# qkniep/alpenglow

Measured on AMD Instinct MI355X. Metric: GiB/s device-resident RS shred encode+reconstruct, batched 1 MiB blocks, higher is better.
Workload: dtype u8 (GF(2^16) symbols, bitsliced u32 planes); 1 GPU; 4096 x 1 MiB blocks per GPU, 32:32 encode + reconstruct with 16/32 data shreds erased; blocks_per_gpu=4096, block_bytes=1048576, data_shreds=32, coding_shreds=32, erased_data_shreds=16, lost_coding_shreds=0, random_patterns=False, parallelism=blocks sharded over 1 GPU(s), no collective, only=both

## Files before the change

### alpenglow_amd/csrc/rs_api.cpp

```cpp
#include <hip/hip_runtime.h>

#include <algorithm>
#include <chrono>
#include <cstddef>
#include <cstdlib>
#include <cstring>
#include <new>
#include <utility>
#include <vector>

#include "../../include/alpenglow_rs.h"
#include "gf16.hpp"
#include "rs_ctx.hpp"
#include "rs_launch.hpp"
#include "rs_patterns.hpp"

using namespace ag::host;
using ag::lowrate_chunk;
using ag::mc_chunk;
using ag::padded_shard;
using ag::xform_points;

namespace {

// ... 218 lines not shown
  return AG_RS_OK;
}

int ag_rs_ctx_set_stream(ag_rs_ctx* c, void* s) {
  if (!c) return AG_RS_ERR_INVALID_ARGUMENT;
  return switch_stream(c, static_cast<hipStream_t>(s));
}

int ag_rs_ctx_reset_stream(ag_rs_ctx* c) {
  if (!c) return AG_RS_ERR_INVALID_ARGUMENT;
  return switch_stream(c, c->own_stream);
}

void* ag_rs_ctx_stream(ag_rs_ctx* c) { return c ? static_cast<void*>(c->stream) : nullptr; }

int ag_rs_ctx_synchronize(ag_rs_ctx* c) {
  if (!c) return AG_RS_ERR_INVALID_ARGUMENT;
  if (c->enter()) return AG_RS_ERR_DEVICE;
  return hipStreamSynchronize(c->stream) == hipSuccess ? AG_RS_OK : AG_RS_ERR_DEVICE;
}

int ag_rs_use_high_rate(size_t k, size_t m) {
  const int hr = ag::use_high_rate(k, m);
  return hr < 0 ? -AG_RS_ERR_UNSUPPORTED_SHARD_COUNT : hr;
}

int ag_rs_internal_last_decode_classes(ag_rs_ctx* c, uint64_t* out16) {
  if (!c || !out16) return AG_RS_ERR_INVALID_ARGUMENT;
  std::memcpy(out16, c->last_classes, sizeof c->last_classes);
  return AG_RS_OK;
}

int ag_rs_internal_last_window_kernels(ag_rs_ctx* c, uint32_t* out) {
  if (!c || !out) return AG_RS_ERR_INVALID_ARGUMENT;
  *out = c->last_window_kernels;
  return AG_RS_OK;
}

int ag_rs_internal_server_jobs(ag_rs_ctx* c, uint64_t* out4) {
  if (!c || !out4) return AG_RS_ERR_INVALID_ARGUMENT;
  std::copy(std::begin(c->server_jobs), std::end(c->server_jobs), out4);
  return AG_RS_OK;
}

int ag_rs_internal_fail_next_server_job(ag_rs_ctx* c) {
  if (!c) return AG_RS_ERR_INVALID_ARGUMENT;
  c->fail_next_server_job = true;
  return AG_RS_OK;
}

int ag_rs_internal_last_encode_kernels(ag_rs_ctx* c, uint32_t* out) {
  if (!c || !out) return AG_RS_ERR_INVALID_ARGUMENT;
  *out = c->last_encode_kernels;
  return AG_RS_OK;
}

int ag_rs_internal_last_merkle_kernels(ag_rs_ctx* c, uint32_t* out) {
  if (!c || !out) return AG_RS_ERR_INVALID_ARGUMENT;
  *out = c->last_merkle_kernels;
  return AG_RS_OK;
}

int ag_rs_internal_last_exact_rerun(ag_rs_ctx* c, uint64_t out[2]) {
  if (!c || !out) return AG_RS_ERR_INVALID_ARGUMENT;
  out[0] = c->last_rerun_slices;
  out[1] = c->last_rerun_passes;
  return AG_RS_OK;
}

int ag_rs_has_fast_path(size_t k, size_t m, size_t S) {
  if (S == 0 || S % 2) return 0;
  const size_t Sp = padded_shard(S);
  return xform_points(k, m, Sp) || mc_chunk(k, m, Sp) || lowrate_chunk(k, m, Sp) ? 1 : 0;
}

int ag_rs_encode_batch(ag_rs_ctx* c, size_t k, size_t m, size_t S, size_t nblocks, const uint8_t* orig,
                       size_t ostride, uint8_t* rec, size_t rstride, int memory) {
  if (!c || (nblocks && (!orig || !rec))) return AG_RS_ERR_INVALID_ARGUMENT;
  int st = check_geometry(k, m, S);
  if (st) return st;
  if (ostride < k * S || rstride < m * S) return AG_RS_ERR_INVALID_ARGUMENT;
  if ((st = c->enter())) return st;
  c->last_encode_kernels = 0;
  if (memory == AG_RS_MEM_DEVICE) return encode_device(c, k, m, S, nblocks, orig, ostride, rec, rstride);
  if (memory != AG_RS_MEM_HOST) return AG_RS_ERR_INVALID_ARGUMENT;
  const size_t in_b = k * S, out_b = m * S;
  const size_t group = std::max<size_t>(1, kStageGroupBytes / (in_b + out_b));
  if ((st = c->ensure_copy_streams())) return st;
  size_t g = 0;
  for (size_t b0 = 0; b0 < nblocks; b0 += group, ++g) {
    const size_t n = std::min(group, nblocks - b0);
    auto& sl = c->slot[g & 1];
    AG_HIP(hipStreamWaitEvent(c->h2d, sl.down, 0));
    if ((st = sl.in.ensure(group * in_b, c->h2d)) || (st = sl.out.ensure(group * out_b, c->h2d))) return st;
    AG_HIP(hipMemcpy2DAsync(sl.in.ptr, in_b, orig + b0 * ostride, ostride, in_b, n, hipMemcpyHostToDevice, c->h2d));
    AG_HIP(hipEventRecord(sl.up, c->h2d));
    AG_HIP(hipStreamWaitEvent(c->stream, sl.up, 0));
    if ((st = encode_device(c, k, m, S, n, sl.in.as<uint8_t>(), in_b, sl.out.as<uint8_t>(), out_b))) break;
    AG_HIP(hipEventRecord(sl.done, c->stream));
    AG_HIP(hipStreamWaitEvent(c->d2h, sl.done, 0));
    AG_HIP(hipMemcpy2DAsync(rec + b0 * rstride, rstride, sl.out.ptr, out_b, out_b, n, hipMemcpyDeviceToHost, c->d2h));
    AG_HIP(hipEventRecord(sl.down, c->d2h));
  }
  AG_HIP(hipStreamSynchronize(c->stream));
  AG_HIP(hipStreamSynchronize(c->d2h));
  return st;
// ... 302 lines not shown
```

### alpenglow_amd/csrc/rs_ctx.hpp

```cpp
#pragma once
#include <hip/hip_runtime.h>

#include <chrono>
#include <cstddef>
#include <cstdint>
#include <memory>
#include <type_traits>
#include <utility>
#include <vector>

#include "../../include/alpenglow_rs.h"
#include "cipher.hpp"
#include "gf16.hpp"
#include "rs_launch.hpp"

#define AG_HIP(expr)                                  \
  do {                                                \
    if ((expr) != hipSuccess) return AG_RS_ERR_DEVICE; \
  } while (0)

namespace ag {
namespace host __attribute__((visibility("hidden"))) {

struct DevBuf {
// ... 113 lines not shown
  template <typename T>
  int host(size_t bytes, T** out) {
    if (ev) AG_HIP(hipEventSynchronize(ev));
    else AG_HIP(hipEventCreateWithFlags(&ev, hipEventDisableTiming));
    const int st = pin.ensure(bytes);
    *out = pin.as<T>();
    return st;
  }
  int send(size_t bytes, hipStream_t stream, void* dst = nullptr) {
    if (!dst) {
      const int st = dev.ensure(bytes, stream);
      if (st) return st;
      dst = dev.ptr;
    }
    AG_HIP(hipMemcpyAsync(dst, pin.ptr, bytes, hipMemcpyHostToDevice, stream));
    AG_HIP(hipEventRecord(ev, stream));
    return AG_RS_OK;
  }
};

}
}

using ag::host::DevBuf;
using ag::host::PinBuf;
using ag::host::StagedUpload;
using ag::host::UploadCache;

struct ag_rs_ctx {
  int device = 0;
  hipStream_t own_stream = nullptr;
  hipStream_t stream = nullptr;
  bool tables_ready = false;
  DevBuf d_exp, d_log, d_skew, d_log_walsh;
  DevBuf scratch;
  DevBuf d_flags, d_loc, d_blocks;
  UploadCache<uint64_t> mask;
  UploadCache<uint64_t> stage_mask;
  UploadCache<uint64_t> xmask;
  size_t xmask_w = 0;
  bool xmask_poly = false;
  DevBuf d_rows, d_xblocks;
  UploadCache<uint64_t> x128;
  DevBuf d_rows128;
  std::vector<uint32_t> x128_ids;
  UploadCache<uint8_t> syn;
  DevBuf d_synblocks;
  UploadCache<uint8_t> corr;
  DevBuf d_corrk, d_corrblocks;
  static constexpr int kClassSlots = 16;
  uint64_t last_classes[kClassSlots] = {};
  int decode_depth = 0;
  uint32_t last_encode_kernels = 0;
  uint32_t last_window_kernels = 0;
  DevBuf d_empty_roots;
  DevBuf d_merkle_nodes;
  uint32_t last_merkle_kernels = 0;
  StagedUpload leaf_sizes;
  StagedUpload block_meta;
  DevBuf d_aon_lens, d_aon_digests, d_aon_keys;
  DevBuf d_aon_lens2;
  hipStream_t side = nullptr;
  hipEvent_t side_fork = nullptr, side_join = nullptr;
  DevBuf d_slice_meta;
  DevBuf stage_pad;
  StagedUpload lens;
  DevBuf d_strip;
  DevBuf d_reenc_mask;
  DevBuf d_pipe_few, d_pipe_mask;
  StagedUpload present;
  PinBuf h_strip;
  PinBuf h_slice_meta;
  PinBuf h_pipe_meta;
  StagedUpload rerun;
  uint64_t last_rerun_slices = 0, last_rerun_passes = 0;
  DevBuf d_ed_base;
  static constexpr int kPipeBufs = 37;
  DevBuf pipe[kPipeBufs];
  DevBuf d_sh_roots, d_sh_commit, d_sh_onvalid, d_sh_list;
  DevBuf d_intake;
  StagedUpload intake_win;
  PinBuf h_intake;
  DevBuf d_repair;
  StagedUpload repair_blocks;
  PinBuf h_repair;
  DevBuf d_block;
  StagedUpload block_cols;
  PinBuf h_block;
  struct Slot {
    DevBuf in, out;
    hipEvent_t up = nullptr, done = nullptr, down = nullptr;
  } slot[2];
  hipStream_t h2d = nullptr, d2h = nullptr;
  DevBuf one_in, one_out;
  ag::LatencyMailbox* mb = nullptr;
  ag::LatencyMailbox* mb_dev = nullptr;
  hipStream_t server_stream = nullptr;
  uint32_t server_seq = 0;
  uint32_t server_p_seq = 0, server_dp_seq = 0;
  bool server_broken = false;
  bool fail_next_server_job = false;
  uint64_t server_jobs[4] = {};
  std::vector<PinBuf> abandoned_pins;

  void forget_uploads() {
    mask.key.clear();
    stage_mask.key.clear();
    xmask.key.clear();
    x128.key.clear();
    syn.key.clear();
    corr.key.clear();
  }

  int enter() { return hipSetDevice(device) == hipSuccess ? AG_RS_OK : AG_RS_ERR_DEVICE; }

  int ensure_tables() {
    if (tables_ready) return AG_RS_OK;
    const ag::Gf16Tables& t = ag::gf16_tables();
    std::vector<uint16_t> lw(t.log, t.log + ag::kGfOrder);
    lw[0] = 0;
    for (size_t dist = 1; dist < ag::kGfOrder; dist <<= 1)
      for (size_t r = 0; r < ag::kGfOrder; r += 2 * dist)
        for (size_t i = r; i < r + dist; ++i) {
          const uint32_t a = lw[i], b = lw[i + dist];
          const uint32_t s = a + b, d = a - b;
          lw[i] = static_cast<uint16_t>(s + (s >> 16));
          lw[i + dist] = static_cast<uint16_t>(d + (d >> 16));
        }
    int st;
    if ((st = d_exp.ensure(sizeof t.exp, stream)) || (st = d_log.ensure(sizeof t.log, stream)) ||
        (st = d_skew.ensure(sizeof t.skew, stream)) || (st = d_log_walsh.ensure(lw.size() * 2, stream)))
      return st;
    AG_HIP(hipMemcpy(d_exp.ptr, t.exp, sizeof t.exp, hipMemcpyHostToDevice));
    AG_HIP(hipMemcpy(d_log.ptr, t.log, sizeof t.log, hipMemcpyHostToDevice));
    AG_HIP(hipMemcpy(d_skew.ptr, t.skew, sizeof t.skew, hipMemcpyHostToDevice));
    AG_HIP(hipMemcpy(d_log_walsh.ptr, lw.data(), lw.size() * 2, hipMemcpyHostToDevice));
    tables_ready = true;
    return AG_RS_OK;
  }

  ag::GfDeviceTables dtables() const {
    return {d_exp.as<uint16_t>(), d_log.as<uint16_t>(), d_skew.as<uint16_t>(), d_log_walsh.as<uint16_t>()};
  }

  int ensure_side_stream() {
    if (side) return AG_RS_OK;
    AG_HIP(hipStreamCreateWithFlags(&side, hipStreamNonBlocking));
    AG_HIP(hipEventCreateWithFlags(&side_fork, hipEventDisableTiming));
    AG_HIP(hipEventCreateWithFlags(&side_join, hipEventDisableTiming));
    return AG_RS_OK;
  }

  int ensure_copy_streams() {
    if (h2d) return AG_RS_OK;
    AG_HIP(hipStreamCreateWithFlags(&h2d, hipStreamNonBlocking));
    AG_HIP(hipStreamCreateWithFlags(&d2h, hipStreamNonBlocking));
    for (Slot& s : slot) {
      AG_HIP(hipEventCreateWithFlags(&s.up, hipEventDisableTiming));
      AG_HIP(hipEventCreateWithFlags(&s.done, hipEventDisableTiming));
      AG_HIP(hipEventCreateWithFlags(&s.down, hipEventDisableTiming));
      AG_HIP(hipEventRecord(s.down, d2h));
    }
    return AG_RS_OK;
  }

  void server_stop() {
    if (!mb) return;
    (void)hipSetDevice(device);
// ... 130 lines not shown
```

### alpenglow_amd/csrc/rs_dispatch.cpp

```cpp
#include <hip/hip_runtime.h>

#include <algorithm>
#include <cstring>
#include <vector>

#include "gf16.hpp"
#include "rs_ctx.hpp"
#include "rs_launch.hpp"
#include "rs_patterns.hpp"
#include "shredder.hpp"

namespace ag {
namespace host {

int check_geometry(size_t k, size_t m, size_t S) {
  if (use_high_rate(k, m) < 0) return AG_RS_ERR_UNSUPPORTED_SHARD_COUNT;
  if (S == 0 || S % 2) return AG_RS_ERR_INVALID_SHARD_SIZE;
  if (S > 0xFFFFFFFEull) return AG_RS_ERR_INVALID_ARGUMENT;
  return AG_RS_OK;
}

bool odd_layout(const void* a, const void* b, size_t sa, size_t sb) {
  return ((reinterpret_cast<uintptr_t>(a) | reinterpret_cast<uintptr_t>(b) | sa | sb) & 1) != 0;
}
// ... 13 lines not shown
  p.rec = rec;
  p.rec_block_stride = rstride;
  p.rec_shard_stride = sstride;
  return p;
}

XformParams xform_params(const uint8_t* in, size_t in_stride, size_t n_in, uint8_t* out, size_t out_stride,
                         size_t n_out, size_t sstride, size_t cps, size_t nblocks) {
  XformParams p{};
  p.in = in;
  p.in_block_stride = in_stride;
  p.in_shard_stride = sstride;
  p.out = out;
  p.out_block_stride = out_stride;
  p.out_shard_stride = sstride;
  p.n_in = static_cast<uint32_t>(n_in);
  p.n_out = static_cast<uint32_t>(n_out);
  p.chunks_per_shard = static_cast<uint32_t>(cps);
  p.total_columns = static_cast<uint64_t>(nblocks) * cps;
  return p;
}

int encode_restrided(ag_rs_ctx* c, size_t k, size_t m, size_t Sv, size_t sstride, size_t off, size_t nblocks,
                     const uint8_t* orig, size_t ostride, uint8_t* rec, size_t rstride) {
  const size_t Sp = padded_shard(Sv), per_block = (k + m) * Sp;
  const size_t group = std::max<size_t>(1, kRestrideGroupBytes / per_block);
  int st = c->stage_pad.ensure(std::min(group, nblocks) * per_block, c->stream);
  if (st) return st;
  c->last_encode_kernels |= kEkRestride;
  uint8_t* pad = c->stage_pad.as<uint8_t>();
  for (size_t b0 = 0; b0 < nblocks; b0 += group) {
    const size_t nb = std::min(group, nblocks - b0);
    if (launch_restride(orig + b0 * ostride + off, ostride, sstride, pad, per_block, Sp, static_cast<uint32_t>(Sv),
                        static_cast<uint32_t>(k), nb, false, nullptr, false, c->stream) != hipSuccess)
      return AG_RS_ERR_DEVICE;
    if ((st = encode_device(c, k, m, Sp, nb, pad, per_block, pad + k * Sp, per_block))) return st;
    if (launch_restride(pad + k * Sp, per_block, Sp, rec + b0 * rstride + off, rstride, sstride,
                        static_cast<uint32_t>(Sv), static_cast<uint32_t>(m), nb, true, nullptr, false,
                        c->stream) != hipSuccess)
      return AG_RS_ERR_DEVICE;
  }
  return AG_RS_OK;
}

int encode_cols(ag_rs_ctx* c, size_t k, size_t m, size_t S, size_t sstride, size_t nblocks, const uint8_t* orig,
                size_t ostride, uint8_t* rec, size_t rstride) {
  const unsigned npts = xform_points(k, m, S);
  const unsigned mc = mc_chunk(k, m, S);
  const unsigned lr = lowrate_chunk(k, m, S);
  if (npts || mc || lr) {
    const XformParams p = xform_params(orig, ostride, k, rec, rstride, m, sstride, S / 64, nblocks);
    hipError_t e = hipSuccess;
    if (npts) {
      c->last_encode_kernels |= npts == 32 ? encode32_kernel(p) : kEkXformH8;
      e = launch_xform(npts == 32 ? XformKind::kEncode32 : XformKind::kEncode64, p, c->stream);
    } else if (mc) {
      c->last_encode_kernels |= kEkEncodeMc;
      e = launch_encode_mc(mc, p, c->stream);
    } else {
      for (size_t j = 0; j * lr < m && e == hipSuccess;) {
        XformParams pj = p;
        pj.out = rec + j * lr * sstride;
        if (lr == 32 && j % 2 == 0 && (j + 1) * lr < m && j < 4) {
          pj.n_out = static_cast<uint32_t>(std::min<size_t>(2 * lr, m - j * lr));
          c->last_encode_kernels |= kEkLowRate2;
          e = launch_xform_lowrate2(static_cast<unsigned>(j / 2), pj, c->stream);
          j += 2;
          continue;
        }
        pj.n_out = static_cast<uint32_t>(std::min<size_t>(lr, m - j * lr));
        c->last_encode_kernels |= kEkLowRate;
        e = launch_xform_lowrate(lr, static_cast<unsigned>(j), pj, c->stream);
        ++j;
      }
    }
    return e == hipSuccess ? AG_RS_OK : AG_RS_ERR_DEVICE;
  }
  int st = c->ensure_tables();
  if (st) return st;
  const int hr = use_high_rate(k, m);
  const size_t chunk = hr ? next_pow2(m) : next_pow2(k);
  const size_t cover = hr ? k : m;
  const size_t rows = std::max(chunk, (cover + chunk - 1) / chunk * chunk);
  const size_t nsym = S / 2;
  const size_t per_block = rows * nsym * 2;
  const size_t per_launch = std::max<size_t>(1, kGenericScratchBytes / per_block);
  if ((st = c->scratch.ensure(std::min(per_launch, nblocks) * per_block, c->stream))) return st;
  for (size_t b0 = 0; b0 < nblocks; b0 += per_launch) {
    auto p = shard_params<GenericEncodeParams>(orig + b0 * ostride, ostride, rec + b0 * rstride, rstride, sstride);
    p.k = static_cast<uint32_t>(k);
    p.m = static_cast<uint32_t>(m);
    p.high_rate = static_cast<uint32_t>(hr);
    p.chunk = static_cast<uint32_t>(chunk);
    p.rows = static_cast<uint32_t>(rows);
    p.shard_bytes = static_cast<uint32_t>(S);
    p.nsym = static_cast<uint32_t>(nsym);
    p.nblocks = std::min(per_launch, nblocks - b0);
    p.scratch = c->scratch.as<uint16_t>();
    p.t = c->dtables();
    c->last_encode_kernels |= kEkGeneric;
    if (launch_generic_encode(p, c->stream) != hipSuccess) return AG_RS_ERR_DEVICE;
  }
  return AG_RS_OK;
}

XformParams tail_params(const uint8_t* in, size_t in_stride, size_t n_in, uint8_t* out, size_t out_stride,
                        size_t n_out, size_t S, size_t nblocks) {
  XformParams p = xform_params(in, in_stride, n_in, out, out_stride, n_out, S, padded_shard(S) / 64, nblocks);
// ... 544 lines not shown
```

### alpenglow_amd/csrc/rs_launch.hpp

```cpp
#pragma once
#include <hip/hip_runtime.h>

#include <cstdint>

namespace ag {

struct XformParams {
  const uint8_t* in;
  uint64_t in_block_stride;
  uint64_t in_shard_stride;
  uint8_t* out;
  uint64_t out_block_stride;
  uint64_t out_shard_stride;
  const uint64_t* out_mask;
  uint32_t pattern_per_block;
  uint32_t n_in;
  uint32_t n_out;
  uint32_t chunks_per_shard;
  uint64_t total_columns;
  uint32_t out_low_half;
  uint32_t skip_idle;
  uint32_t tail_bytes;
};

enum class XformKind { kEncode32, kDecode32, kEncode64, kDecode64 };

enum EncodeKernelBit : uint32_t {
  kEkXform4 = 1u << 0,
  kEkXform8 = 1u << 1,
  kEkXformH8 = 1u << 2,
  kEkEncodeMc = 1u << 3,
  kEkLowRate = 1u << 4,
  kEkLowRate2 = 1u << 5,
  kEkGeneric = 1u << 6,
  kEkRestride = 1u << 7,
  kEkVar = 1u << 8,
};
inline EncodeKernelBit encode32_kernel(const XformParams& p) {
  const uint64_t groups = (p.total_columns + 63) / 64;
  return groups < 256 || p.chunks_per_shard == 128 || p.chunks_per_shard == 256 ? kEkXform8 : kEkXform4;
}

hipError_t launch_xform(XformKind kind, const XformParams& p, hipStream_t stream);
bool xform_supported(unsigned n);
hipError_t launch_xform64(unsigned din, unsigned dout, const XformParams& p, hipStream_t stream);
hipError_t launch_xform_lowrate(unsigned n, unsigned j, const XformParams& p, hipStream_t stream);
hipError_t launch_xform_lowrate2(unsigned pair, const XformParams& p, hipStream_t stream);
hipError_t launch_xform_lowrate_decode(unsigned j, const XformParams& p, hipStream_t stream);
hipError_t launch_encode_mc(unsigned chunk, const XformParams& p, hipStream_t stream);

struct SynPattern {
  uint64_t dmask;
  uint32_t e;
  uint8_t rec[4];
  uint8_t out[4];
  uint32_t pad;
  uint32_t rows[4][4][16];
};
struct DecodeSynParams {
  const uint8_t* rec;
  uint64_t rec_block_stride;
  uint64_t rec_shard_stride;
  uint8_t* orig;
  uint64_t orig_block_stride;
  uint64_t orig_shard_stride;
  const SynPattern* pat;
  const uint32_t* block_ids;
  uint32_t per_block;
  uint32_t tiles_per_block;
  uint32_t k;
  uint32_t chunks_per_shard;
  uint64_t total_columns;
  uint64_t ntiles;
};
hipError_t launch_decode_syn(unsigned chunk, const DecodeSynParams& p, hipStream_t stream);

constexpr int kCorrMaxSyn = 16;
constexpr int kCorrMaxPairs = 256;
constexpr int kCorrPairWords = 64;
struct CorrPattern {
  uint64_t rmask;
  uint64_t emask;
  uint64_t smask;
  uint32_t ne, ns;
  uint64_t kofs;
  uint32_t wsum[8];
  uint32_t wslot[8][4];
};
struct DecodeCParams {
  const uint8_t* rec;
  uint64_t rec_block_stride;
  uint64_t rec_shard_stride;
  uint8_t* orig;
  uint64_t orig_block_stride;
  uint64_t orig_shard_stride;
  const CorrPattern* pat;
// ... 147 lines not shown
```

### alpenglow_amd/csrc/rs_tile64.hip

```cpp
#include <hip/hip_runtime.h>

#include "rs_decode_pk.hpp"
#include "rs_device.hpp"
#include "rs_launch.hpp"
#include "rs_xform.hpp"
#include "rs_xform8.hpp"

namespace ag {
namespace {

using dev::static_for;

template <int DIN, int DOUT, int TAIL = 0>
__global__ __launch_bounds__(256, 2) void xform_kernel(const XformParams p) {
  __shared__ uint4 lds[16 * 4 * kXfLanes];
  const int lane = threadIdx.x & 63;
  const int wave = __builtin_amdgcn_readfirstlane(threadIdx.x >> 6);
  const uint32_t tile = dev::xcd_tile(blockIdx.x, gridDim.x);
  if (p.skip_idle) {
    const uint64_t col = static_cast<uint64_t>(tile) * kXfLanes + lane;
    const uint64_t m = col < p.total_columns ? p.out_mask[col / p.chunks_per_shard] : 0;
    if (__builtin_amdgcn_ballot_w64(m != 0) == 0) return;
  }
  Regs8 ra;
  xf_load_raw<TAIL>(p, tile_io<TAIL>(p, tile, lane, p.in_block_stride), wave, ra);
  uint64_t mask[4] = {~0ull, ~0ull, ~0ull, ~0ull};
  if (p.out_mask) {
    if (!p.pattern_per_block) {
      const uint64_t m = p.out_mask[0];
      mask[0] = mask[1] = mask[2] = mask[3] = m;
    } else {
      const TileIO io = tile_io<TAIL>(p, tile, lane, p.out_block_stride);
      static_for<4>([&](auto Q) {
        constexpr int q = decltype(Q)::value;
        mask[q] = p.out_mask[io.blk[q]];
      });
    }
  }

  if constexpr (TAIL == 1) {
    const TileIO in_io = tile_io<TAIL>(p, tile, lane, p.in_block_stride);
    static_for<8>([&](auto T) { tail_fix_all<TAIL>(in_io, ra[decltype(T)::value]); });
  }
  static_for<8>([&](auto T) {
    swap_halves(ra[decltype(T)::value]);
    dev::planes_from_raw(ra[decltype(T)::value]);
  });
  xf_pass_a<DIN>(wave, ra);
  Regs8 rb;
  xf_exchange_ab(wave, lane, lds, ra, rb);
  xf_pass_b<DIN, DOUT>(rb);
  xf_exchange_bc(wave, lane, lds, rb, ra);

  const TileIO out_io = tile_io<TAIL>(p, tile, lane, p.out_block_stride);
  const uint32_t qall = qmask_all<8>(out_io, mask, 8 * wave, p.n_out);
  if (__builtin_amdgcn_ballot_w64(qall != 0) == 0) return;
  xf_pass_c<DOUT>(wave, ra);
  static_for<8>([&](auto T) {
    constexpr int t = decltype(T)::value;
    const uint32_t s = 8 * wave + t;
    const uint32_t q = (qall >> (4 * t)) & 15u;
    if (s < p.n_out && __builtin_amdgcn_ballot_w64(q != 0) != 0)
      store_shard<false, TAIL>(p.out + s * p.out_shard_stride, out_io, q, ra[t]);
  });
}

template <int DIN, int DOUT, bool HALF = false, int TAIL = 0>
__global__ __launch_bounds__(512, 4) void xform8_kernel(const XformParams p) {
  __shared__ uint4 lds[16 * 4 * kXfLanes];
  __shared__ X8Flags flags;
  if (threadIdx.x < 16) reinterpret_cast<uint32_t*>(&flags)[threadIdx.x] = 0;
  __syncthreads();
  xform8_tile<DIN, DOUT, HALF, TAIL>(p, dev::xcd_tile(blockIdx.x, gridDim.x), lds, &flags);
}

template <int DIN, int DOUT, bool HALF>
__global__ __launch_bounds__(512, 4) void xform8_stream_kernel(const XformParams p) {
  __shared__ uint4 lds[16 * 4 * kXfLanes];
  __shared__ X8Flags flags;
  if (threadIdx.x < 16) reinterpret_cast<uint32_t*>(&flags)[threadIdx.x] = 0;
  __syncthreads();
  xform8_stream_tile<DIN, DOUT, HALF>(p, dev::xcd_tile(blockIdx.x, gridDim.x), lds, &flags);
}


__device__ __forceinline__ void mul_rt4(uint32_t* x, const uint32_t* __restrict__ rows) {
  uint32_t t0[16], t1[16], t2[16], t3[16];
  auto build = [&](uint32_t* t, uint32_t a, uint32_t b, uint32_t c, uint32_t d) {
    t[0] = 0;
    t[1] = a;
    t[2] = b;
    t[3] = a ^ b;
    t[4] = c;
    t[5] = a ^ c;
    t[6] = b ^ c;
    t[7] = dev::xor3(a, b, c);
    t[8] = d;
    t[9] = a ^ d;
    t[10] = b ^ d;
    t[11] = dev::xor3(a, b, d);
    t[12] = c ^ d;
    t[13] = dev::xor3(a, c, d);
    t[14] = dev::xor3(b, c, d);
    t[15] = dev::xor3(t[3], c, d);
  };
  build(t0, x[0], x[1], x[2], x[3]);
  build(t1, x[4], x[5], x[6], x[7]);
  build(t2, x[8], x[9], x[10], x[11]);
  build(t3, x[12], x[13], x[14], x[15]);
  static_for<16>([&](auto O) {
    constexpr int o = decltype(O)::value;
    const uint32_t r = __builtin_amdgcn_readfirstlane(rows[o]);
    x[o] = dev::xor3(t0[r & 15], t1[(r >> 4) & 15], t2[(r >> 8) & 15]) ^ t3[(r >> 12) & 15];
  });
}

__device__ __forceinline__ void xf_derivative(int wave, int lane, uint4* lds, Regs8& r) {
// ... 476 lines not shown
    }
  });
  static_for<C>([&](auto A) {
    constexpr int a = decltype(A)::value;
    if (a < e) store_shard(p.orig + sp->out[a] * p.orig_shard_stride, io, io.valid, out[a]);
  });
}

}

bool xform_supported(unsigned n) { return n == 32 || n == 64; }

hipError_t launch_xform_lowrate(unsigned n, unsigned j, const XformParams& p, hipStream_t stream) {
  if (p.total_columns == 0) return hipSuccess;
  const uint64_t tiles = (p.total_columns + 63) / 64;
  if (tiles > 0x7FFFFFFFull) return hipErrorInvalidValue;
  const dim3 grid(static_cast<unsigned>(tiles));
  if (n == 32) {
    switch (j) {
      case 0: hipLaunchKernelGGL((xform_kernel<0, 32>), grid, dim3(256), 0, stream, p); break;
      case 1: hipLaunchKernelGGL((xform_kernel<0, 64>), grid, dim3(256), 0, stream, p); break;
      case 2: hipLaunchKernelGGL((xform_kernel<0, 96>), grid, dim3(256), 0, stream, p); break;
      case 3: hipLaunchKernelGGL((xform_kernel<0, 128>), grid, dim3(256), 0, stream, p); break;
      default: return hipErrorInvalidValue;
    }
  } else if (n == 64) {
    switch (j) {
      case 0: return launch_xform64(0, 64, p, stream);
      case 1: return launch_xform64(0, 128, p, stream);
      case 2: return launch_xform64(0, 192, p, stream);
      default: return hipErrorInvalidValue;
    }
  } else {
    return hipErrorInvalidValue;
  }
  return hipGetLastError();
}

hipError_t launch_xform_lowrate_decode(unsigned j, const XformParams& p, hipStream_t stream) {
  if (p.total_columns == 0) return hipSuccess;
  const uint64_t tiles = (p.total_columns + 63) / 64;
  if (tiles > 0x7FFFFFFFull) return hipErrorInvalidValue;
  const dim3 grid(static_cast<unsigned>(tiles));
  switch (j) {
    case 0: hipLaunchKernelGGL((xform_kernel<32, 0>), grid, dim3(256), 0, stream, p); break;
    case 1: hipLaunchKernelGGL((xform_kernel<64, 0>), grid, dim3(256), 0, stream, p); break;
    case 2: hipLaunchKernelGGL((xform_kernel<96, 0>), grid, dim3(256), 0, stream, p); break;
    case 3: hipLaunchKernelGGL((xform_kernel<128, 0>), grid, dim3(256), 0, stream, p); break;
    default: return hipErrorInvalidValue;
  }
  return hipGetLastError();
}

hipError_t launch_xform(XformKind kind, const XformParams& p, hipStream_t stream) {
  if (p.total_columns == 0) return hipSuccess;
  const uint64_t groups = (p.total_columns + kXfLanes - 1) / kXfLanes;
  if (groups > 0x7FFFFFFFull) return hipErrorInvalidValue;
  const dim3 grid(static_cast<unsigned>(groups));
  switch (kind) {
    case XformKind::kEncode32:
      if (p.tail_bytes) {
        if (encode32_kernel(p) == kEkXform8)
          hipLaunchKernelGGL((xform8_kernel<32, 0, false, 1>), grid, dim3(512), 0, stream, p);
        else
          hipLaunchKernelGGL((xform_kernel<32, 0, 1>), grid, dim3(256), 0, stream, p);
        break;
      }
      if (encode32_kernel(p) == kEkXform8)
        hipLaunchKernelGGL((xform8_kernel<32, 0>), grid, dim3(512), 0, stream, p);
      else
        hipLaunchKernelGGL((xform_kernel<32, 0>), grid, dim3(256), 0, stream, p);
      break;
    case XformKind::kDecode32:
      if (p.tail_bytes) {
        if (p.out_low_half)
          hipLaunchKernelGGL((xform8_kernel<0, 32, true, 1>), grid, dim3(512), 0, stream, p);
        else
          hipLaunchKernelGGL((xform8_kernel<0, 32, false, 1>), grid, dim3(512), 0, stream, p);
        break;
      }
      if (p.n_in == 32 && p.out_mask) {
        if (p.out_low_half)
          hipLaunchKernelGGL((xform8_stream_kernel<0, 32, true>), grid, dim3(512), 0, stream, p);
        else
          hipLaunchKernelGGL((xform8_stream_kernel<0, 32, false>), grid, dim3(512), 0, stream, p);
        break;
      }
      if (p.out_low_half)
        hipLaunchKernelGGL((xform8_kernel<0, 32, true>), grid, dim3(512), 0, stream, p);
      else
        hipLaunchKernelGGL((xform8_kernel<0, 32>), grid, dim3(512), 0, stream, p);
      break;
    case XformKind::kEncode64:
      return launch_xform64(64, 0, p, stream);
    case XformKind::kDecode64:
      return launch_xform64(0, 64, p, stream);
    default:
      return hipErrorInvalidValue;
  }
  return hipGetLastError();
}

hipError_t launch_decode_x32(bool per_lane, dim3 grid, const DecodeXParams& p, hipStream_t stream) {
  if (per_lane) hipLaunchKernelGGL((decode_x_kernel<true>), grid, dim3(256), 0, stream, p);
  else hipLaunchKernelGGL((decode_x_kernel<>), grid, dim3(256), 0, stream, p);
  return hipGetLastError();
}

hipError_t launch_decode_x16(int pass, unsigned din, unsigned dout, dim3 grid, const DecodeXParams& p,
                             hipStream_t stream) {
#define AG_X16(PS, DI, DO) hipLaunchKernelGGL((decode_x16_kernel<PS, DI, DO>), grid, dim3(1024), 0, stream, p)
  if (pass == 0 && din == 0 && dout == 0) AG_X16(0, 0, 0);
  else if (pass == 1 && din == 64 && dout == 0) AG_X16(1, 64, 0);
  else if (pass == 2 && din == 0 && dout == 0) AG_X16(2, 0, 0);
  else if (pass == 1 && din == 0 && dout == 64) AG_X16(1, 0, 64);
  else if (pass == 2 && din == 64 && dout == 64) AG_X16(2, 64, 64);
  else return hipErrorInvalidValue;
#undef AG_X16
  return hipGetLastError();
}

hipError_t launch_encode_mc(unsigned chunk, const XformParams& p, hipStream_t stream) {
// ... 170 lines not shown
```

### alpenglow_amd/csrc/rs_xform.hpp

```cpp
#pragma once
#include <hip/hip_runtime.h>

#include <type_traits>

#include "rs_device.hpp"
#include "rs_launch.hpp"
#include "unaligned.hpp"

namespace ag {
namespace {

using dev::static_for;


constexpr int kXfLanes = 64;

using Regs8 = uint32_t[8][16];

template <int S, bool INV>
__device__ __forceinline__ void bfly(uint32_t* x, uint32_t* y) {
  if constexpr (INV) dev::ifft_bfly<S>(x, y); else dev::fft_bfly<S>(x, y);
}
template <int BASE, bool INV>
__device__ __forceinline__ void bfly_w(int wave, uint32_t* x, uint32_t* y) {
// ... 364 lines not shown
template <int TAIL>
__device__ __forceinline__ void st_piece_io(uint8_t* base, const TileIO& io, int q, uint32_t a, uint32_t b, uint32_t c,
                                            uint32_t d) {
  st_piece(base + io.off[q], a, b, c, d);
}

__device__ __forceinline__ void swap_halves(uint32_t* v) {
  static_for<8>([&](auto K) {
    constexpr int k = decltype(K)::value;
    const auto r = __builtin_amdgcn_permlane32_swap(v[k], v[k + 8], false, false);
    v[k] = r[0];
    v[k + 8] = r[1];
  });
}

template <int TAIL = 0>
__device__ __forceinline__ void xf_load_raw(const XformParams& p, const TileIO& io, int wave, Regs8& raw) {
  static_for<8>([&](auto T) {
    constexpr int t = decltype(T)::value;
    const uint32_t s = 8 * wave + t;
    if (s < p.n_in) {
      const uint8_t* base = p.in + s * p.in_shard_stride;
      static_for<4>([&](auto Q) {
        constexpr int q = decltype(Q)::value;
        const uint4 x = ld_piece_io<TAIL>(base, io, q);
        raw[t][4 * q] = x.x;
        raw[t][4 * q + 1] = x.y;
        raw[t][4 * q + 2] = x.z;
        raw[t][4 * q + 3] = x.w;
      });
    } else {
      static_for<16>([&](auto P) { raw[t][decltype(P)::value] = 0; });
    }
  });
}

template <int NS>
__device__ __forceinline__ void load_slots_stream(const XformParams& p, const TileIO& io, uint32_t s0,
                                                  uint32_t (*raw)[16]) {
  static_for<NS>([&](auto T) {
    constexpr int t = decltype(T)::value;
    const uint8_t* base = p.in + (s0 + t) * p.in_shard_stride;
    static_for<4>([&](auto Q) {
      constexpr int q = decltype(Q)::value;
      const uint4 x = ld_piece(base + io.off[q]);
      raw[t][4 * q] = x.x;
      raw[t][4 * q + 1] = x.y;
      raw[t][4 * q + 2] = x.z;
      raw[t][4 * q + 3] = x.w;
    });
  });
}

template <bool ACC = false, int TAIL = 0>
__device__ __forceinline__ void store_shard(uint8_t* __restrict__ base, const TileIO& io, uint32_t qmask,
                                            const uint32_t* planes) {
  uint32_t v[16];
  static_for<16>([&](auto P) {
    constexpr int i = decltype(P)::value;
    v[i] = planes[i];
  });
  dev::transpose8(v);
  dev::transpose8(v + 8);
  swap_halves(v);
  if constexpr (TAIL == 1) {
    const int lane = threadIdx.x & 63;
    static_for<4>([&](auto Q) {
      constexpr int q = decltype(Q)::value;
      if (__builtin_amdgcn_ballot_w64((io.tailq >> q) & 1) != 0) {
        uint32_t w[4] = {v[4 * q], v[4 * q + 1], v[4 * q + 2], v[4 * q + 3]};
        tail_window(w, lane, io.tlen_h);
        if ((io.tailq >> q) & 1) {
          static_for<4>([&](auto K) { v[4 * q + decltype(K)::value] = w[decltype(K)::value]; });
          if (io.tlen == 0) qmask &= ~(1u << q);
        }
      }
    });
  }
  static_for<4>([&](auto Q) {
    constexpr int q = decltype(Q)::value;
    if (qmask & (1u << q)) {
      if constexpr (ACC) {
        static_assert(TAIL != 1, "accumulating stores of tail windows are not supported");
        const uint4 x = ld_piece_io<TAIL>(base, io, q);
        uint32_t o[4] = {x.x, x.y, x.z, x.w};
        st_piece_io<TAIL>(base, io, q, v[4 * q] ^ o[0], v[4 * q + 1] ^ o[1], v[4 * q + 2] ^ o[2], v[4 * q + 3] ^ o[3]);
      } else {
        st_piece_io<TAIL>(base, io, q, v[4 * q], v[4 * q + 1], v[4 * q + 2], v[4 * q + 3]);
      }
    }
  });
}

__device__ __forceinline__ void xf_exchange_ab(int wave, int lane, uint4* lds, Regs8& ra, Regs8& rb) {
  static_for<2>([&](auto Rho) {
    constexpr int rho = decltype(Rho)::value;
    static_for<4>([&](auto U) {
      constexpr int u = decltype(U)::value;
      lds_put(lds, 4 * wave + u, lane, ra[4 * rho + u]);
    });
    __syncthreads();
    static_for<4>([&](auto W2) {
      constexpr int w2 = decltype(W2)::value;
      lds_get(lds, 4 * w2 + wave, lane, rb[2 * w2 + rho]);
    });
    __syncthreads();
// ... 303 lines not shown
```

### alpenglow_amd/rs.py

```python

from __future__ import annotations

import ctypes
import os
from dataclasses import dataclass

LIB_PATH = os.path.join(os.path.dirname(os.path.abspath(__file__)), "_lib",
                        os.environ.get("AG_RS_LIB_NAME", "libalpenglow_rs.so"))

MEM_DEVICE = 0
MEM_HOST = 1
DECODE_EXACT = 0
DECODE_ANY_K = 1

DATA_SHREDS = 32
TOTAL_SHREDS = 64
MAX_DATA_PER_SHRED = 1024
MAX_DATA_PER_SLICE = DATA_SHREDS * MAX_DATA_PER_SHRED - 1

STATUS_KIND = {
    1: "InvalidShardSize",
    2: "DifferentShardSize",
    3: "TooFewOriginalShards",
    4: "TooManyOriginalShards",
# ... 92 lines not shown
        "ag_rs_decoder_add_recovery_shard": ([p, sz, p, sz], i),
        "ag_rs_decoder_decode": ([p], i),
        "ag_rs_decoder_restored_original": ([p, sz, pp, psz], i),
        "ag_rs_decoder_free": ([p], None),
        "ag_rs_coder_new": ([p, sz, pp], i),
        "ag_rs_encoder_new_on_device": ([i, sz, sz, sz, pp], i),
        "ag_rs_decoder_new_on_device": ([i, sz, sz, sz, pp], i),
        "ag_rs_coder_new_on_device": ([i, sz, pp], i),
        "ag_rs_coder_free": ([p], None),
        "ag_rs_coder_num_coding": ([p, psz], i),
        "ag_rs_coder_shred": ([p, p, sz, p, p, psz], i),
        "ag_rs_coder_deshred": ([p, sz, p, p, p, p, psz, p, p, psz], i),
        "ag_rs_coder_shred_batch": ([p, sz, sz, sz, p, sz, p, p, sz], i),
        "ag_rs_coder_deshred_batch": ([p, sz, sz, sz, p, sz, p, p, i, p], i),
        "ag_rs_coder_shred_bytes": ([sz, psz], i),
        "ag_rs_coder_shred_batch_var": ([p, sz, sz, p, sz, p, p, sz, p], i),
        "ag_rs_coder_deshred_batch_var": ([p, sz, sz, p, p, sz, p, p, i, p], i),
        "ag_merkle_empty_root": ([sz, p], i),
        "ag_merkle_height": ([sz], sz),
        "ag_merkle_node_count": ([sz], sz),
        "ag_merkle_build_batch": ([p, sz, sz, sz, p, sz, sz, p, p, sz, p, sz], i),
        "ag_merkle_build_batch_var": ([p, sz, p, p, sz, p, p, sz, p, sz], i),
        "ag_merkle_verify_batch": ([p, sz, sz, p, sz, p, p, sz, p, sz, sz, p], i),
        "ag_block_tree_batch": ([p, sz, p, p, p, p, sz, p, sz], i),
        "ag_block_proof_check_batch": ([p, sz, p, sz, p, p, sz, p, sz, p, p, p], i),
        "ag_aes128_encrypt_block": ([p, p, p], i),
        "ag_cipher_apply_keystream_batch": ([p, sz, p, p, sz, p], i),
        "ag_sha256_batch": ([p, sz, p, sz, p, p], i),
        "ag_aon_encrypt_batch": ([p, i, sz, p, p, sz, p], i),
        "ag_aon_decrypt_batch": ([p, i, sz, p, sz, p, p], i),
        "ag_ed25519_public_key_batch": ([p, sz, p, p], i),
        "ag_ed25519_sign_batch": ([p, sz, p, sz, p, sz, p, sz, sz, p], i),
        "ag_ed25519_verify_batch": ([p, sz, p, sz, p, sz, p, sz, p, sz, p], i),
        "ag_shred_validate_batch": ([p, sz, p, sz, sz, p, p, sz, sz, p, p, p, p, sz, p, p, p, p, p, p], i),
        "ag_slice_sign_batch": ([p, sz, p, p, p, p, p, p, p, p], i),
        "ag_shred_deserialize_batch": ([p, sz, p, sz, p, p, p], i),
        "ag_shred_serialize_batch": ([p, sz, p, p, sz, p], i),
        "ag_shred_datagram_bytes": ([sz, sz, psz], i),
        "ag_slice_frame_batch": ([p, sz, sz, p, p, p, sz, p, p, sz, p], i),
        "ag_slice_parse_batch": ([p, sz, p, sz, p, p, p, p, p, p], i),
        "ag_shredder_shred_batch": ([p, sz, sz, p, p, p, sz, p, p, p, p, p, p, p, p, p, p, sz, p], i),
        "ag_shredder_deshred_batch": ([p, sz, sz, p, sz, p, p, p, p, p, p, p, p, p, p, p], i),
        "ag_shredder_shred_batch_var": ([p, sz, p, p, p, sz, p, p, p, p, p, p, p, sz, p, p, p, p, sz, p, sz, p, p], i),
        "ag_shredder_shred_batch_kind": ([p, i, sz, sz, p, p, p, sz, p, p, p, p, p, p, p, p, sz, p, p, p, sz, p], i),
        "ag_shredder_deshred_batch_kind": ([p, i, sz, sz, p, sz, p, p, p, sz, p, p, p, p, p, p, p, p], i),
        "ag_shredder_deshred_batch_var": ([p, sz, p, p, sz, p, p, p, sz, p, p, p, p, p, p, p, p], i),
        "ag_shredder_intake_batch": ([p, sz, p, sz, sz, p, sz, p, p, p, sz, p, p, p, p, p, p, p], i),
        "ag_repair_intake_batch": ([p, sz, p, p, sz, sz, p, sz, p, p, p, p, p, p, p, sz, p, p, p, p, p, p, p, p], i),
        "ag_block_assemble_batch": ([p, sz, sz, p, p, p, p, p, p, sz, p, sz, p, sz, p, p, p, p, p, p, p, p, sz, p, sz,
                                     p, p, sz, p, p], i),
    }
    sigs["ag_rs_internal_last_decode_classes"] = ([p, p], i)
    sigs["ag_rs_internal_last_encode_kernels"] = ([p, p], i)
    sigs["ag_rs_internal_fail_next_server_job"] = ([p], i)
    sigs["ag_rs_internal_server_jobs"] = ([p, p], i)
    sigs["ag_rs_internal_last_window_kernels"] = ([p, p], i)
    sigs["ag_rs_internal_last_merkle_kernels"] = ([p, p], i)
    sigs["ag_rs_internal_last_exact_rerun"] = ([p, p], i)
    for name, (args, res) in sigs.items():
        if not hasattr(L, name):
            continue
        f = getattr(L, name)
        f.argtypes = args
        f.restype = res
    _lib = L
    return L


def _check(status: int, where: str):
    if status != 0:
        raise RSError(status, where)


def use_high_rate(k: int, m: int) -> bool:
    r = load().ag_rs_use_high_rate(k, m)
    if r < 0:
        raise RSError(-r, "use_high_rate")
    return bool(r)


def has_fast_path(k: int, m: int, shard_bytes: int) -> bool:
    return bool(load().ag_rs_has_fast_path(k, m, shard_bytes))


def device_count() -> int:
    n = ctypes.c_int(0)
    load().ag_rs_device_count(ctypes.byref(n))
    return n.value


def _split(buf, S: int, n: int) -> list:
    raw = ctypes.string_at(buf, S * n)
    return [raw[i * S:(i + 1) * S] for i in range(n)]


_pycoder = None


def _coder_binding():
    global _pycoder
    if _pycoder is None:
        import importlib.util
        import sysconfig

        path = os.path.join(os.path.dirname(LIB_PATH), "_pycoder" + (sysconfig.get_config_var("EXT_SUFFIX") or ".so"))
        mod = False
# ... 140 lines not shown
    lens = np.ascontiguousarray(np.asarray(payload_lens, dtype=np.uint32))
    if lens.size != nslices:
        raise ValueError("payload_lens does not match the batch")
    out = np.zeros(nslices, np.uint32)
    _check(load().ag_rs_coder_shred_batch_var(ctx.handle, num_coding, nslices,
                                              _ptr(payloads) if payloads is not None else None, payload_stride,
                                              lens.ctypes.data, _ptr(codewords), codeword_stride, out.ctypes.data),
           "ag_rs_coder_shred_batch_var")
    return out


def coder_deshred_batch_var(ctx: Context, num_coding: int, nslices: int, shred_bytes, codewords,
                            codeword_stride: int, data_present, coding_present,
                            mode: int = DECODE_EXACT, as_array: bool = False):
    import numpy as np

    sizes = np.ascontiguousarray(np.asarray(shred_bytes, dtype=np.uint32))
    dp = np.ascontiguousarray(np.frombuffer(bytes(data_present), np.uint8) if isinstance(data_present, (bytes, bytearray))
                              else np.asarray(data_present, dtype=np.uint8))
    cp = np.ascontiguousarray(np.frombuffer(bytes(coding_present), np.uint8) if isinstance(coding_present, (bytes, bytearray))
                              else np.asarray(coding_present, dtype=np.uint8))
    if sizes.size != nslices or dp.size != nslices * 32 or cp.size != nslices * num_coding:
        raise ValueError("shred sizes / present-flag arrays do not match the batch")
    out = np.empty(nslices, np.int64)
    _check(load().ag_rs_coder_deshred_batch_var(ctx.handle, num_coding, nslices, sizes.ctypes.data, _ptr(codewords),
                                                codeword_stride, dp.ctypes.data, cp.ctypes.data, mode,
                                                out.ctypes.data),
           "ag_rs_coder_deshred_batch_var")
    if as_array:
        return out
    return [int(v) if v >= 0 else STATUS_KIND.get(int(-v), f"Status{int(-v)}") for v in out]


DECODE_CLASSES = {0: "none", 1: "transform", 2: "generic", 3: "window64", 4: "syndrome", 5: "lowrate_chunk",
                  6: "correction", 8: "window128", 9: "server_window64"}


def last_decode_classes(ctx: Context) -> dict:
    import numpy as np

    out = np.zeros(16, np.uint64)
    _check(load().ag_rs_internal_last_decode_classes(ctx.handle, out.ctypes.data), "last_decode_classes")
    return {DECODE_CLASSES.get(i, str(i)): int(v) for i, v in enumerate(out) if v}


ENCODE_KERNELS = ("xform4", "xform8", "xform_h8", "encode_mc", "lowrate", "lowrate2", "generic", "restride",
                  "var_encode")


def last_encode_kernels(ctx: Context) -> set:
    out = ctypes.c_uint32(0)
    _check(load().ag_rs_internal_last_encode_kernels(ctx.handle, ctypes.byref(out)), "last_encode_kernels")
    return {name for i, name in enumerate(ENCODE_KERNELS) if out.value >> i & 1}


WINDOW_KERNELS = ("decode_pk_fused", "decode_pk", "decode_h8_fused", "decode_h8", "decode_x16", "var_decode")


def last_window_kernels(ctx: Context) -> set:
    out = ctypes.c_uint32(0)
    _check(load().ag_rs_internal_last_window_kernels(ctx.handle, ctypes.byref(out)), "last_window_kernels")
    return {name for i, name in enumerate(WINDOW_KERNELS) if out.value >> i & 1}


SERVER_JOBS = ("encode32", "decode32", "decode32_half", "decode_pk")


def server_jobs(ctx: Context) -> dict:
    import numpy as np

    out = np.zeros(4, np.uint64)
    _check(load().ag_rs_internal_server_jobs(ctx.handle, out.ctypes.data), "server_jobs")
    return dict(zip(SERVER_JOBS, (int(v) for v in out)))


def fail_next_server_job(ctx: Context):
    _check(load().ag_rs_internal_fail_next_server_job(ctx.handle), "fail_next_server_job")


def fill_splitmix(ctx: Context, device_dst, nblocks: int, block_bytes: int, dst_block_stride: int,
                  seed_base: int):
    _check(load().ag_rs_fill_splitmix(ctx.handle, _ptr(device_dst), nblocks, block_bytes,
                                      dst_block_stride, seed_base), "ag_rs_fill_splitmix")



class ReedSolomonEncoder:

    def __init__(self, ctx: Context | None, original_count: int, recovery_count: int, shard_bytes: int,
                 device: int = 0):
        self._lib = load()
        self.ctx = ctx
        h = ctypes.c_void_p()
        if ctx is None:
            st = self._lib.ag_rs_encoder_new_on_device(device, original_count, recovery_count, shard_bytes,
                                                       ctypes.byref(h))
        else:
            st = self._lib.ag_rs_encoder_new(ctx.handle, original_count, recovery_count, shard_bytes,
                                             ctypes.byref(h))
        _check(st, "ReedSolomonEncoder::new")
        self.handle = h
        self.recovery_count = recovery_count

    def reset(self, original_count: int, recovery_count: int, shard_bytes: int):
        _check(self._lib.ag_rs_encoder_reset(self.handle, original_count, recovery_count, shard_bytes),
               "ReedSolomonEncoder::reset")
# ... 690 lines not shown
```

Before: 1606 GiB/s.

## Add persistent staged encode32 kernel prefetching next tile into LDS

Adds a persistent-grid variant of the 32:32 encode transform, sized to twice the CU count by default. Each workgroup loops over tiles and uses global_load_lds to prefetch half of the next tile's input slots into LDS while the current tile's later passes and stores run, so memory latency overlaps with compute. The kernel is used only for the xform4 path with full-width, untailed, unmasked geometry. A persistent grid may lose some latency hiding compared with the oversubscribed launch, and the LDS staging adds synchronisation constraints.

```diff
diff --git a/alpenglow_amd/csrc/rs_api.cpp b/alpenglow_amd/csrc/rs_api.cpp
--- a/alpenglow_amd/csrc/rs_api.cpp
+++ b/alpenglow_amd/csrc/rs_api.cpp
@@ -294,6 +294,14 @@
 int ag_rs_internal_last_encode_kernels(ag_rs_ctx* c, uint32_t* out) {
   if (!c || !out) return AG_RS_ERR_INVALID_ARGUMENT;
   *out = c->last_encode_kernels;
+  return AG_RS_OK;
+}
+
+int ag_rs_internal_last_encode_bits(ag_rs_ctx* c, uint32_t* out) { return ag_rs_internal_last_encode_kernels(c, out); }
+
+int ag_rs_internal_set_staged_grid(ag_rs_ctx* c, uint32_t workgroups) {
+  if (!c) return AG_RS_ERR_INVALID_ARGUMENT;
+  c->staged_cap = workgroups;
   return AG_RS_OK;
 }
 
diff --git a/alpenglow_amd/csrc/rs_ctx.hpp b/alpenglow_amd/csrc/rs_ctx.hpp
--- a/alpenglow_amd/csrc/rs_ctx.hpp
+++ b/alpenglow_amd/csrc/rs_ctx.hpp
@@ -189,6 +189,8 @@
   uint64_t last_classes[kClassSlots] = {};
   int decode_depth = 0;
   uint32_t last_encode_kernels = 0;
+  uint32_t staged_cap = 0;
+  uint32_t cu_count = 0;
   uint32_t last_window_kernels = 0;
   DevBuf d_empty_roots;
   DevBuf d_merkle_nodes;
@@ -251,6 +253,17 @@
 
   int enter() { return hipSetDevice(device) == hipSuccess ? AG_RS_OK : AG_RS_ERR_DEVICE; }
 
+  int staged_grid(uint32_t* out) {
+    if (!cu_count) {
+      int n = 0;
+      AG_HIP(hipDeviceGetAttribute(&n, hipDeviceAttributeMultiprocessorCount, device));
+      if (n <= 0) return AG_RS_ERR_DEVICE;
+      cu_count = static_cast<uint32_t>(n);
+    }
+    *out = staged_cap ? staged_cap : 2 * cu_count;
+    return AG_RS_OK;
+  }
+
   int ensure_tables() {
     if (tables_ready) return AG_RS_OK;
     const ag::Gf16Tables& t = ag::gf16_tables();
diff --git a/alpenglow_amd/csrc/rs_dispatch.cpp b/alpenglow_amd/csrc/rs_dispatch.cpp
--- a/alpenglow_amd/csrc/rs_dispatch.cpp
+++ b/alpenglow_amd/csrc/rs_dispatch.cpp
@@ -89,8 +89,12 @@
     const XformParams p = xform_params(orig, ostride, k, rec, rstride, m, sstride, S / 64, nblocks);
     hipError_t e = hipSuccess;
     if (npts) {
-      c->last_encode_kernels |= npts == 32 ? encode32_kernel(p) : kEkXformH8;
-      e = launch_xform(npts == 32 ? XformKind::kEncode32 : XformKind::kEncode64, p, c->stream);
+      uint32_t staged = 0;
+      if (npts == 32 && encode32_staged(p)) {
+        if (const int st = c->staged_grid(&staged)) return st;
+      }
+      c->last_encode_kernels |= npts == 32 ? encode32_kernel(p) | (staged ? kEkStaged : 0u) : kEkXformH8;
+      e = launch_xform(npts == 32 ? XformKind::kEncode32 : XformKind::kEncode64, p, c->stream, staged);
     } else if (mc) {
       c->last_encode_kernels |= kEkEncodeMc;
       e = launch_encode_mc(mc, p, c->stream);
diff --git a/alpenglow_amd/csrc/rs_launch.hpp b/alpenglow_amd/csrc/rs_launch.hpp
--- a/alpenglow_amd/csrc/rs_launch.hpp
+++ b/alpenglow_amd/csrc/rs_launch.hpp
@@ -35,13 +35,18 @@
   kEkGeneric = 1u << 6,
   kEkRestride = 1u << 7,
   kEkVar = 1u << 8,
+  kEkStaged = 1u << 9,
 };
 inline EncodeKernelBit encode32_kernel(const XformParams& p) {
   const uint64_t groups = (p.total_columns + 63) / 64;
   return groups < 256 || p.chunks_per_shard == 128 || p.chunks_per_shard == 256 ? kEkXform8 : kEkXform4;
 }
-
-hipError_t launch_xform(XformKind kind, const XformParams& p, hipStream_t stream);
+inline bool encode32_staged(const XformParams& p) {
+  return encode32_kernel(p) == kEkXform4 && p.tail_bytes == 0 && p.n_in == 32 && p.n_out == 32 && !p.out_mask &&
+         p.total_columns % 64 == 0;
+}
+
+hipError_t launch_xform(XformKind kind, const XformParams& p, hipStream_t stream, uint32_t staged_grid = 0);
 bool xform_supported(unsigned n);
 hipError_t launch_xform64(unsigned din, unsigned dout, const XformParams& p, hipStream_t stream);
 hipError_t launch_xform_lowrate(unsigned n, unsigned j, const XformParams& p, hipStream_t stream);
diff --git a/alpenglow_amd/csrc/rs_tile64.hip b/alpenglow_amd/csrc/rs_tile64.hip
--- a/alpenglow_amd/csrc/rs_tile64.hip
+++ b/alpenglow_amd/csrc/rs_tile64.hip
@@ -1,4 +1,6 @@
 #include <hip/hip_runtime.h>
+
+#include <algorithm>
 
 #include "rs_decode_pk.hpp"
 #include "rs_device.hpp"
@@ -63,6 +65,58 @@
     if (s < p.n_out && __builtin_amdgcn_ballot_w64(q != 0) != 0)
       store_shard<false, TAIL>(p.out + s * p.out_shard_stride, out_io, q, ra[t]);
   });
+}
+
+constexpr uint32_t kNoTile = ~0u;
+template <bool STAGED>
+__device__ __forceinline__ void xform_staged_tile(const XformParams& p, uint32_t tile, uint32_t next, int wave, int lane,
+                                                  uint4* lds) {
+  const TileIO io = tile_io_g(p.total_columns, p.chunks_per_shard, tile, lane, p.in_block_stride);
+  Regs8 ra;
+  if constexpr (STAGED) {
+    load_slots_stream<4>(p, io, 8 * wave + 4, ra + 4);
+    staged_get4<16>(lds, 4 * wave, lane, ra);
+  } else {
+    load_slots_stream<8>(p, io, 8 * wave, ra);
+  }
+  static_for<8>([&](auto T) {
+    swap_halves(ra[decltype(T)::value]);
+    dev::planes_from_raw(ra[decltype(T)::value]);
+  });
+  xf_pass_a<32>(wave, ra);
+  Regs8 rb;
+  xf_exchange_ab(wave, lane, lds, ra, rb);
+  xf_pass_b<32, 0>(rb);
+  xf_exchange_bc(wave, lane, lds, rb, ra);
+  if (next != kNoTile) {
+    __asm__ volatile("s_waitcnt lgkmcnt(0)" ::: "memory");
+    const TileIO nio = tile_io_g(p.total_columns, p.chunks_per_shard, next, lane, p.in_block_stride);
+    stage_slots_lds<4>(p, nio, 8 * wave, lds, 4 * wave);
+  }
+  xf_pass_c<0>(wave, ra);
+  const TileIO out_io = tile_io_g(p.total_columns, p.chunks_per_shard, tile, lane, p.out_block_stride);
+  static_for<8>([&](auto T) {
+    constexpr int t = decltype(T)::value;
+    store_shard<false, 0>(p.out + (8 * wave + t) * p.out_shard_stride, out_io, 15u, ra[t]);
+  });
+}
+
+__global__ __launch_bounds__(256, 2) void xform_staged_kernel(const XformParams p) {
+  __shared__ uint4 lds[16 * 4 * kXfLanes];
+  const int lane = threadIdx.x & 63;
+  const int wave = __builtin_amdgcn_readfirstlane(threadIdx.x >> 6);
+  const uint32_t tiles = static_cast<uint32_t>(p.total_columns / kXfLanes);
+  uint32_t i = blockIdx.x;
+  if (i >= tiles) return;
+  auto tile_at = [&](uint32_t j) { return j < tiles ? dev::xcd_tile(j, tiles) : kNoTile; };
+  uint32_t tile = tile_at(i), next = tile_at(i + gridDim.x);
+  xform_staged_tile<false>(p, tile, next, wave, lane, lds);
+  while (next != kNoTile) {
+    i += gridDim.x;
+    tile = next;
+    next = tile_at(i + gridDim.x);
+    xform_staged_tile<true>(p, tile, next, wave, lane, lds);
+  }
 }
 
 template <int DIN, int DOUT, bool HALF = false, int TAIL = 0>
@@ -645,7 +699,7 @@
   return hipGetLastError();
 }
 
-hipError_t launch_xform(XformKind kind, const XformParams& p, hipStream_t stream) {
+hipError_t launch_xform(XformKind kind, const XformParams& p, hipStream_t stream, uint32_t staged_grid) {
   if (p.total_columns == 0) return hipSuccess;
   const uint64_t groups = (p.total_columns + kXfLanes - 1) / kXfLanes;
   if (groups > 0x7FFFFFFFull) return hipErrorInvalidValue;
@@ -661,6 +715,8 @@
       }
       if (encode32_kernel(p) == kEkXform8)
         hipLaunchKernelGGL((xform8_kernel<32, 0>), grid, dim3(512), 0, stream, p);
+      else if (staged_grid && encode32_staged(p))
+        hipLaunchKernelGGL(xform_staged_kernel, dim3(std::min(grid.x, staged_grid)), dim3(256), 0, stream, p);
       else
         hipLaunchKernelGGL((xform_kernel<32, 0>), grid, dim3(256), 0, stream, p);
       break;
diff --git a/alpenglow_amd/csrc/rs_xform.hpp b/alpenglow_amd/csrc/rs_xform.hpp
--- a/alpenglow_amd/csrc/rs_xform.hpp
+++ b/alpenglow_amd/csrc/rs_xform.hpp
@@ -440,6 +440,57 @@
   });
 }
 
+typedef __attribute__((address_space(1))) const void* GldsSrc;
+typedef __attribute__((address_space(3))) void* GldsDst;
+template <int NS>
+__device__ __forceinline__ void stage_slots_lds(const XformParams& p, const TileIO& io, uint32_t s0, uint4* lds,
+                                                int slot0) {
+  static_for<NS>([&](auto T) {
+    constexpr int t = decltype(T)::value;
+    const uint8_t* base = p.in + (s0 + t) * p.in_shard_stride;
+    static_for<4>([&](auto Q) {
+      constexpr int q = decltype(Q)::value;
+      __builtin_amdgcn_global_load_lds((GldsSrc)(base + io.off[q]), (GldsDst)(lds + ((slot0 + t) * 4 + q) * kXfLanes), 16,
+                                       0, 2);
+    });
+  });
+}
+template <int N>
+__device__ __forceinline__ void staged_get4(uint4* lds, int slot0, int lane, uint32_t (*raw)[16]) {
+  const uint32_t a = static_cast<uint32_t>(reinterpret_cast<uintptr_t>((GldsDst)(lds + slot0 * 4 * kXfLanes + lane)));
+  dev::u32x4 x[16];
+  __asm__ volatile(
+      "s_waitcnt vmcnt(%17)\n\t"
+      "ds_read_b128 %0, %16\n\t"
+      "ds_read_b128 %1, %16 offset:1024\n\t"
+      "ds_read_b128 %2, %16 offset:2048\n\t"
+      "ds_read_b128 %3, %16 offset:3072\n\t"
+      "ds_read_b128 %4, %16 offset:4096\n\t"
+      "ds_read_b128 %5, %16 offset:5120\n\t"
+      "ds_read_b128 %6, %16 offset:6144\n\t"
+      "ds_read_b128 %7, %16 offset:7168\n\t"
+      "ds_read_b128 %8, %16 offset:8192\n\t"
+      "ds_read_b128 %9, %16 offset:9216\n\t"
+      "ds_read_b128 %10, %16 offset:10240\n\t"
+      "ds_read_b128 %11, %16 offset:11264\n\t"
+      "ds_read_b128 %12, %16 offset:12288\n\t"
+      "ds_read_b128 %13, %16 offset:13312\n\t"
+      "ds_read_b128 %14, %16 offset:14336\n\t"
+      "ds_read_b128 %15, %16 offset:15360\n\t"
+      "s_waitcnt lgkmcnt(0)"
+      : "=&v"(x[0]), "=&v"(x[1]), "=&v"(x[2]), "=&v"(x[3]), "=&v"(x[4]), "=&v"(x[5]), "=&v"(x[6]), "=&v"(x[7]),
+        "=&v"(x[8]), "=&v"(x[9]), "=&v"(x[10]), "=&v"(x[11]), "=&v"(x[12]), "=&v"(x[13]), "=&v"(x[14]), "=&v"(x[15])
+      : "v"(a), "n"(N)
+      : "memory");
+  static_for<16>([&](auto I) {
+    constexpr int i = decltype(I)::value;
+    raw[i >> 2][4 * (i & 3)] = x[i].x;
+    raw[i >> 2][4 * (i & 3) + 1] = x[i].y;
+    raw[i >> 2][4 * (i & 3) + 2] = x[i].z;
+    raw[i >> 2][4 * (i & 3) + 3] = x[i].w;
+  });
+}
+
 template <bool ACC = false, int TAIL = 0>
 __device__ __forceinline__ void store_shard(uint8_t* __restrict__ base, const TileIO& io, uint32_t qmask,
                                             const uint32_t* planes) {
diff --git a/alpenglow_amd/rs.py b/alpenglow_amd/rs.py
--- a/alpenglow_amd/rs.py
+++ b/alpenglow_amd/rs.py
@@ -168,6 +168,8 @@
     }
     sigs["ag_rs_internal_last_decode_classes"] = ([p, p], i)
     sigs["ag_rs_internal_last_encode_kernels"] = ([p, p], i)
+    sigs["ag_rs_internal_last_encode_bits"] = ([p, p], i)
+    sigs["ag_rs_internal_set_staged_grid"] = ([p, ctypes.c_uint32], i)
     sigs["ag_rs_internal_fail_next_server_job"] = ([p], i)
     sigs["ag_rs_internal_server_jobs"] = ([p, p], i)
     sigs["ag_rs_internal_last_window_kernels"] = ([p, p], i)
@@ -414,6 +416,19 @@
     out = ctypes.c_uint32(0)
     _check(load().ag_rs_internal_last_encode_kernels(ctx.handle, ctypes.byref(out)), "last_encode_kernels")
     return {name for i, name in enumerate(ENCODE_KERNELS) if out.value >> i & 1}
+
+
+ENCODE_STAGED = 1 << 9
+
+
+def last_encode_bits(ctx: Context) -> int:
+    out = ctypes.c_uint32(0)
+    _check(load().ag_rs_internal_last_encode_bits(ctx.handle, ctypes.byref(out)), "last_encode_bits")
+    return out.value
+
+
+def set_staged_grid(ctx: Context, workgroups: int = 0):
+    _check(load().ag_rs_internal_set_staged_grid(ctx.handle, workgroups), "set_staged_grid")
 
 
 WINDOW_KERNELS = ("decode_pk_fused", "decode_pk", "decode_h8_fused", "decode_h8", "decode_x16", "var_decode")
```

Result: slower. 1507 GiB/s (-6.1%).
